# jorgeMFS/HYMET

Measured on AMD Instinct MI355X. Metric: contigs/s + Mbp/s classified, CAMI-medium, 1/2/4/8 MI355X; % HBM roofline, higher is better.
Workload: dtype u64

## Files before the change

hymet_amd/_lib.py:

```python
from __future__ import annotations

import ctypes
import os

HERE = os.path.dirname(os.path.abspath(__file__))
LIB_PATH = os.path.join(HERE, "libhymet_gpu.so")

_c = ctypes
_i64, _u64, _i32, _u32, _vp = _c.c_int64, _c.c_uint64, _c.c_int, _c.c_uint32, _c.c_void_p

_SIGS = {
    "hymet_version": (_i32, []),
    "hymet_init": (_i32, [_i32, _c.POINTER(_vp)]),
    "hymet_destroy": (_i32, [_vp]),
    "hymet_last_error": (_c.c_char_p, []),
    "hymet_set_stream": (_i32, [_vp, _vp]),
    "hymet_sync": (_i32, [_vp]),
    "hymet_prof_enable": (_i32, [_vp, _i32]),
    "hymet_prof_reset": (_i32, [_vp]),
    "hymet_prof_query": (_i32, [_vp, _c.c_char_p, _c.POINTER(_c.c_double), _c.POINTER(_i64), _c.POINTER(_c.c_double)]),
    "hymet_prof_names": (_i32, [_vp, _c.c_char_p, _i64]),
    "hymet_scratch_trim": (_i32, [_vp, _c.POINTER(_i64)]),
    "hymet_scratch_cached": (_i32, [_vp, _c.POINTER(_i64)]),
    "hymet_scratch_stats": (_i32, [_vp, _vp]),
# ... 42 lines not shown
    "hymet_paf_acc_create": (_i32, [_vp, _c.POINTER(_vp)]),
    "hymet_paf_acc_reset": (_i32, [_vp]),
    "hymet_paf_acc_destroy": (_i32, [_vp]),
    "hymet_paf_acc_info": (_i32, [_vp, _c.POINTER(_i64), _c.POINTER(_vp), _c.POINTER(_vp), _c.POINTER(_vp),
                                  _c.POINTER(_vp), _c.POINTER(_vp)]),
    "hymet_paf_acc_append": (_i32, [_vp, _vp, _vp, _i64, _i64]),
    "hymet_paf_acc_copy": (_i32, [_vp, _vp, _vp, _vp, _vp]),
    "hymet_paf_acc_field": (_i32, [_vp, _vp, _i32, _vp]),
    "hymet_mm_map_acc": (_i32, [_vp, _vp, _vp, _vp, _vp, _vp, _vp, _vp, _i32, _i32, _i32, _i32, _vp]),
    "hymet_emit_paf": (_i32, [_vp, _vp, _vp, _vp, _vp, _vp, _vp, _vp, _vp, _i64, _c.POINTER(_i64), _vp]),
    "hymet_acc_ref_counts": (_i32, [_vp, _vp, _vp]),
    "hymet_acc_classify": (_i32, [_vp, _vp, _i32, _i32] + [_vp] * 15 + [_c.POINTER(_i32)]),
    "hymet_emit_tsv": (_i32, [_vp, _i32, _i32] + [_vp] * 14 + [_i64, _c.POINTER(_i64)]),
    "hymet_mm_chain_dp": (_i32, [_vp, _vp, _vp, _i64, _i32, _i32, _i32, _i32, _i32, _c.c_float, _c.c_float, _vp, _vp]),
    "hymet_mm_mark_compact": (_i32, [_vp, _vp, _vp, _vp, _i64, _vp, _vp, _i32, _vp, _vp, _vp, _c.POINTER(_i64)]),
    "hymet_mm_anchor_sort": (_i32, [_vp, _vp, _vp, _i64, _vp, _i32, _i32, _i32, _u64, _i64, _vp, _vp, _vp, _vp, _vp]),
    "hymet_lca_ref_counts": (_i32, [_vp, _vp, _i64, _vp]),
    "hymet_lca": (_i32, [_vp, _i32, _i32] + [_vp] * 17),
}

_lib = None
_oom_hook = None


def _release_torch_cache(_user):
    try:
        import torch
        torch.cuda.empty_cache()
    except Exception:
        pass
# ... 134 lines not shown
```

hymet_amd/csrc/common.hpp:

```cpp
#pragma once
#include <hip/hip_runtime.h>
#include <stdint.h>
#include <algorithm>
#include <cstdlib>
#include <map>
#include <string>
#include <utility>
#include <vector>
#include "../../include/hymet_gpu.h"

struct hymet_ctx {
    int device = 0;
    hipStream_t stream = nullptr;
    bool own_stream = false;
    int n_cu = 256;
    bool prof = false;
    std::map<std::string, std::vector<std::pair<hipEvent_t, hipEvent_t>>> ev;
    std::map<std::string, double> bytes;
    std::map<std::string, std::pair<int, double>> dev_bytes;
    int64_t *prof_dev = nullptr;
    void *stage[2] = {nullptr, nullptr};
    hipEvent_t stage_ev[2] = {nullptr, nullptr};
    int64_t *mbox_h = nullptr;
    int64_t *mbox_d = nullptr;
    int32_t *dctr = nullptr;
};

namespace hymet {
struct ProfScope {
    hymet_ctx *c;
    const char *name;
    hipEvent_t a = nullptr, b = nullptr;
    ProfScope(hymet_ctx *ctx, const char *n, double alg_bytes = 0.0) : c(ctx), name(n) {
        if (c && c->prof && hipEventCreate(&a) == hipSuccess && hipEventCreate(&b) == hipSuccess) {
            (void)hipEventRecord(a, c->stream);
            c->bytes[name] += alg_bytes;
        }
    }
    ProfScope(hymet_ctx *ctx, const char *n, int slot, double per_unit) : ProfScope(ctx, n, 0.0) {
        if (c && c->prof) c->dev_bytes[name] = {slot, per_unit};
// ... 26 lines not shown
}
inline int64_t env_int(const char *name, int64_t dflt, int64_t lo, int64_t hi) {
    const char *e = env_str(name);
    return e ? std::max(lo, std::min(hi, (int64_t)atoll(e))) : dflt;
}
}

namespace hymet {
void set_error(const std::string &msg);
int fail(int code, const std::string &msg);
int hip_fail(hipError_t e, const char *what);
inline int64_t cdiv(int64_t a, int64_t b) { return (a + b - 1) / b; }
hipError_t scratch_alloc(size_t bytes, hipStream_t stream, void **p, size_t *cls);
void set_oom_hook(void (*hook)(void *), void *user);
void scratch_free(void *p, hipStream_t stream, size_t cls);
}

#define HY_CHECK_LAUNCH(what)                                   \
    do {                                                        \
        hipError_t e_ = hipGetLastError();                      \
        if (e_ != hipSuccess) return hymet::hip_fail(e_, what); \
    } while (0)

#define HY_HIP(call)                                            \
    do {                                                        \
        hipError_t e_ = (call);                                 \
        if (e_ != hipSuccess) return hymet::hip_fail(e_, #call); \
    } while (0)

#define HY_ARG(cond, msg)                                                   \
// ... 4 lines not shown
```

hymet_amd/csrc/ctx.cpp:

```cpp
#include "common.hpp"

#include <algorithm>
#include <thread>
#include <vector>

#include <cstring>
#include <map>
#include <mutex>
#include <tuple>
#include <cstdlib>
#include <vector>

namespace hymet {
static thread_local std::string g_err;
void set_error(const std::string &msg) { g_err = msg; }
int fail(int code, const std::string &msg) {
    g_err = msg;
    return code;
}
int hip_fail(hipError_t e, const char *what) {
    g_err = std::string(what) + ": " + hipGetErrorString(e);
    return HYMET_E_HIP;
}

// ... 98 lines not shown
    g_cache[{dev, stream, cls}].push_back(p);
    g_cached += cls;
}

int scratch_trim(int dev, int64_t *freed) {
    std::lock_guard<std::mutex> lk(g_cache_mu);
    const size_t before = g_cached;
    drop_cached(dev);
    if (freed) *freed = (int64_t)(before - g_cached);
    return HYMET_OK;
}

int64_t scratch_cached() {
    std::lock_guard<std::mutex> lk(g_cache_mu);
    return (int64_t)g_cached;
}

void scratch_stats(int64_t *out) {
    std::lock_guard<std::mutex> lk(g_cache_mu);
    for (int k = 0; k < 3; k++) out[k] = g_stats[k];
}
}

extern "C" {

int hymet_version(void) { return 1; }

const char *hymet_last_error(void) { return hymet::g_err.c_str(); }

int hymet_init(int device, hymet_ctx **out) {
// ... 27 lines not shown
        return hymet::fail(HYMET_E_HIP, "hymet_init: counter allocation failed");
    }
    *out = c;
    return HYMET_OK;
}

int hymet_destroy(hymet_ctx *ctx) {
    if (!ctx) return HYMET_OK;
    (void)hipSetDevice(ctx->device);
    for (int k = 0; k < 2; k++) {
        if (ctx->stage[k]) (void)hipHostFree(ctx->stage[k]);
        if (ctx->stage_ev[k]) (void)hipEventDestroy(ctx->stage_ev[k]);
    }
    if (ctx->mbox_h) (void)hipHostFree(ctx->mbox_h);
    if (ctx->dctr) (void)hipFree(ctx->dctr);
    if (ctx->prof_dev) (void)hipFree(ctx->prof_dev);
    if (ctx->own_stream && ctx->stream) (void)hipStreamDestroy(ctx->stream);
    delete ctx;
    return HYMET_OK;
}

int hymet_set_stream(hymet_ctx *ctx, void *s) {
    HY_ARG(ctx != nullptr, "hymet_set_stream: null ctx");
    HY_HIP(hipSetDevice(ctx->device));
    if (ctx->own_stream && ctx->stream) (void)hipStreamDestroy(ctx->stream);
    ctx->stream = (hipStream_t)s;
    ctx->own_stream = false;
    return HYMET_OK;
}

int hymet_prof_enable(hymet_ctx *ctx, int on) {
    HY_ARG(ctx != nullptr, "hymet_prof_enable: null ctx");
    ctx->prof = on != 0;
    return HYMET_OK;
}

int hymet_prof_reset(hymet_ctx *ctx) {
    HY_ARG(ctx != nullptr, "hymet_prof_reset: null ctx");
    HY_HIP(hipStreamSynchronize(ctx->stream));
// ... 36 lines not shown
}

int hymet_prof_names(hymet_ctx *ctx, char *buf, int64_t cap) {
    HY_ARG(ctx && buf && cap > 0, "hymet_prof_names: null argument");
    std::string all;
    for (auto &kv : ctx->ev) all += kv.first + "\n";
    if ((int64_t)all.size() + 1 > cap) return hymet::fail(HYMET_E_CAPACITY, "hymet_prof_names: buffer too small");
    memcpy(buf, all.c_str(), all.size() + 1);
    return HYMET_OK;
}

int hymet_scratch_trim(hymet_ctx *ctx, int64_t *freed_bytes) {
    HY_ARG(ctx != nullptr, "hymet_scratch_trim: null ctx");
    HY_HIP(hipSetDevice(ctx->device));
    HY_HIP(hipDeviceSynchronize());
    return hymet::scratch_trim(ctx->device, freed_bytes);
}

int hymet_scratch_reserve(hymet_ctx *ctx, int64_t bytes) {
    HY_ARG(ctx && bytes > 0, "hymet_scratch_reserve: bad argument");
    HY_HIP(hipSetDevice(ctx->device));
    void *p = nullptr;
    size_t cls = 0;
    HY_HIP(hymet::scratch_alloc((size_t)bytes, ctx->stream, &p, &cls));
    hymet::scratch_free(p, ctx->stream, cls);
    return HYMET_OK;
}

int hymet_set_oom_hook(void (*hook)(void *user), void *user) {
    hymet::set_oom_hook(hook, user);
// ... 91 lines not shown
```

hymet_amd/csrc/mm_chain.hip:

```cpp
#include "mm_common.hpp"

#include <cstdlib>
#include <string>

namespace hymet {
namespace mm {
namespace {

#ifndef HYMET_CHAIN_RING
#define HYMET_CHAIN_RING 128
#endif
#ifndef HYMET_CHAIN_SUMRING
#define HYMET_CHAIN_SUMRING 16
#endif
#ifndef HYMET_CHAIN_BDQ
#define HYMET_CHAIN_BDQ 32
#endif
#ifndef HYMET_CHAIN_IDQ
#define HYMET_CHAIN_IDQ 64
#endif
#ifndef HYMET_CHAIN_SPEC_GAP0
#define HYMET_CHAIN_SPEC_GAP0 2
#endif
#ifndef HYMET_CHAIN_WPE
// ... 1285 lines not shown
            ++i;
        }
        if (t_used) {
            __builtin_amdgcn_wave_barrier();
            for (int32_t j = lane; j < n; j += 64) P.t_global[g0 + j] = 0;
        }
        CPROF_FLUSH;
        GTIME_STOP;
    }
}

struct BacktrackParams {
    const int64_t *g_start;
    const int32_t *f;
    const int32_t *p;
    int32_t *t;
    const int32_t *z_cnt;
    const int32_t *z_idx;
    int32_t n_groups;
    int min_cnt, min_sc, max_drop;
    int64_t long_min;
    unsigned long long *prof;
    int32_t *chain_ids;
    uint64_t *chain_u;
    int64_t *chain_first;
    int32_t *n_chains;
};

constexpr int kBtWin = 8;

constexpr int64_t kBtLong = 64;
// ... 503 lines not shown
            hipLaunchKernelGGL(chain_work_anchors_kernel, dim3(wb), dim3(256), 0, st, P.g_start, P.order, P.n_work,
                               (const int32_t *)split.as<int32_t>(), pc);
            HY_CHECK_LAUNCH("chain_work_anchors_kernel");
        }
        P.work_end = split.as<int32_t>();
        if (long_pass) hipLaunchKernelGGL(chain_groups_kernel<1>, dim3((unsigned)blocks), dim3(64), kChainLds, st, P);
        else hipLaunchKernelGGL(chain_groups_kernel<0>, dim3((unsigned)blocks), dim3(64), kChainLds, st, P);
        HY_CHECK_LAUNCH("chain_groups_kernel");
    }
    ProfScope _pl(ctx, long_pass ? "mm_chain_long_small" : "mm_chain_small", slot + 1, 24.0);
    hipLaunchKernelGGL(chain_small_kernel, dim3((unsigned)cdiv(P.n_work, 64)), dim3(64), 0, st, P, (const int32_t *)split.as<int32_t>());
    HY_CHECK_LAUNCH("chain_small_kernel");
    return HYMET_OK;
}

int launch_backtrack(hymet_ctx *ctx, const int64_t *g_start, const int32_t *f, const int32_t *p, int32_t *t,
                     const int32_t *z_cnt, const int32_t *z_idx, int32_t n_groups, const int32_t *order, int32_t n_work,
                     int min_cnt, int min_sc, int max_drop, int32_t *chain_ids, uint64_t *chain_u, int64_t *chain_first,
                     int32_t *n_chains, int64_t n_anchors) {
    if (n_groups <= 0) return HYMET_OK;
    const int64_t long_min = env_int("HYMET_BT_LONG", kBtLong, 0, INT64_MAX);
    const bool prof = env_flag("HYMET_BT_PROF");
    DevBuf pbuf;
    if (prof) {
        HY_HIP(pbuf.alloc(64, ctx->stream));
        HY_HIP(hipMemsetAsync(pbuf.p, 0, 64, ctx->stream));
    }
    BacktrackParams P{g_start,  f,         p,       t,           z_cnt,    z_idx, n_groups, min_cnt, min_sc, max_drop,
                      long_min, (unsigned long long *)pbuf.p, chain_ids, chain_u, chain_first, n_chains};
    DevBuf cnt;
    HY_HIP(cnt.alloc(4 * (size_t)kBtCtrPad * (kBtStripes + 1), ctx->stream));
    ProfScope _ps(ctx, "mm_backtrack", 24.0 * (double)n_anchors);
    if (n_work > 0) {
        hipLaunchKernelGGL(bt_long_count_kernel, dim3(1), dim3(1), 0, ctx->stream, g_start, order, n_work, long_min,
                           cnt.as<int32_t>());
        HY_CHECK_LAUNCH("bt_long_count_kernel");
    }
    hipLaunchKernelGGL(backtrack_groups_kernel, dim3((unsigned)cdiv(n_groups, 64)), dim3(64), 0, ctx->stream, P);
    HY_CHECK_LAUNCH("backtrack_groups_kernel");
    if (n_work > 0) {
        ProfScope _pl(ctx, "mm_backtrack.long");
        const int per_cu = (int)env_int("HYMET_BT_WAVES", 24, 1, 1024);
        const int64_t nb = std::min<int64_t>(n_work, (int64_t)ctx->n_cu * per_cu);
        hipLaunchKernelGGL(backtrack_long_kernel, dim3((unsigned)nb), dim3(64), 0, ctx->stream, P, order,
                           cnt.as<int32_t>(), cnt.as<int32_t>() + kBtCtrPad);
        HY_CHECK_LAUNCH("backtrack_long_kernel");
    }
// ... 13 lines not shown
```

hymet_amd/csrc/mm_chainset.hip:

```cpp
#include "mm_stages.hpp"

#include <algorithm>
#include <cstdio>

namespace hymet {
namespace mm {

int launch_chain(hymet_ctx *ctx, const int32_t *ax, const uint32_t *ay, int span, const int64_t *g_start, const uint8_t *g_qfirst,
                 const int32_t *order, int32_t n_work, int32_t *f, int32_t *p, int32_t *t_global, int max_dist,
                 int max_dist_inner, int bw, int max_chn_skip, int cap_rmq_size, float pen_gap, float pen_skip,
                 int64_t n_anchors, int64_t n_groups);
int launch_backtrack(hymet_ctx *ctx, const int64_t *g_start, const int32_t *f, const int32_t *p, int32_t *t,
                     const int32_t *z_cnt, const int32_t *z_idx, int32_t n_groups, const int32_t *order, int32_t n_work,
                     int min_cnt, int min_sc, int max_drop, int32_t *chain_ids, uint64_t *chain_u, int64_t *chain_first,
                     int32_t *n_chains, int64_t n_anchors);

namespace {

constexpr int kGTile = 16384;

__device__ __forceinline__ uint64_t group_tile_bits(const uint32_t *hb, int64_t n, const int64_t *qoff, int n_q, int64_t t0,
                                                    uint64_t *qs) {
    __shared__ int s_q0;
    const int tid = threadIdx.x;
    const int64_t t1 = min(t0 + kGTile, n);
    const int64_t a0 = t0 + 64 * (int64_t)tid;
    const uint64_t hw = a0 < n ? reinterpret_cast<const uint64_t *>(hb)[a0 >> 6] : 0;
// ... 73 lines not shown
    if ((threadIdx.x & 63) == 0 && i < n) hb[i >> 6] = b;
}

__global__ void max_group_kernel(const int64_t *g_start, const int32_t *order, int32_t G, int64_t *out) {
    if (blockIdx.x != 0 || threadIdx.x != 0) return;
    int64_t best = 0;
    for (int32_t w = 0; w < G; w++) {
        const int g = order[w];
        const int64_t sz = g_start[g + 1] - g_start[g];
        best = max(best, sz);
        if (sz < 0xffff) break;
    }
    *out = best;
}

__global__ void nonwork_fp_kernel(const int64_t *g_start, int32_t G, int min_cnt, int32_t *f, int32_t *p, int32_t *t) {
    const int g = blockIdx.x * blockDim.x + threadIdx.x;
    if (g >= G) return;
    const int64_t a0 = g_start[g], a1 = g_start[g + 1];
    if (a1 - a0 >= min_cnt) return;
    for (int64_t a = a0; a < a1; a++) f[a] = 0, p[a] = -1, t[a] = 0;
}

__global__ void group_size_kernel(const int64_t *g_start, int32_t G, int min_cnt, uint32_t *key, uint32_t *gidx,
                                  uint32_t *is_work, uint8_t *qfirst, int32_t *zlists) {
    const int g = blockIdx.x * blockDim.x + threadIdx.x;
    if (g < 8) zlists[g] = 0;
    if (g >= G) return;
    if (qfirst) qfirst[g] = 0;
    const int64_t sz = g_start[g + 1] - g_start[g];
    key[g] = 0xffffu - (uint32_t)min(sz, (int64_t)0xffff);
    gidx[g] = (uint32_t)g;
    is_work[g] = sz >= min_cnt ? 1u : 0u;
}

constexpr int kZs = 2048;
// ... 408 lines not shown
        int64_t l2 = c, h2 = n_chain - 1;
        while (l2 < h2) {
            const int64_t mid = (l2 + h2 + 1) >> 1;
            if (bpos[mid] <= b) l2 = mid;
            else h2 = mid - 1;
        }
        c = l2;
    }
    const int32_t m = (int32_t)cu[c];
    const int64_t a = chain_ids[cfirst[c] + m - 1 - (b - bpos[c])];
    bx[b] = ax[a];
    by[b] = ay[a];
    bchain[b] = (int32_t)c;
}

__device__ __forceinline__ uint32_t keep_bits16(const int32_t *t, int64_t n, const uint32_t *qflag, const int64_t *qoff,
                                                int n_q, int64_t e0) {
    if (e0 >= n) return 0u;
    int lo = 0, hi = n_q - 1;
    while (lo < hi) {
        const int mid = (lo + hi + 1) >> 1;
        if (qoff[mid] <= e0) lo = mid;
        else hi = mid - 1;
    }
    int q = lo;
    int64_t qend = qoff[q + 1];
    int32_t v[16];
    if (e0 + 16 <= n) {
        const int4 *p4 = reinterpret_cast<const int4 *>(t + e0);
#pragma unroll
        for (int u = 0; u < 4; u++) {
            const int4 w = p4[u];
            v[4 * u] = w.x, v[4 * u + 1] = w.y, v[4 * u + 2] = w.z, v[4 * u + 3] = w.w;
        }
    } else {
#pragma unroll
        for (int u = 0; u < 16; u++) v[u] = e0 + u < n ? t[e0 + u] : 0;
    }
    uint32_t bits = 0, fl = qflag[q];
#pragma unroll
    for (int u = 0; u < 16; u++) {
        while (e0 + u >= qend && q + 1 < n_q) {
            q++;
            qend = qoff[q + 1];
            fl = qflag[q];
        }
        bits |= (uint32_t)(v[u] == 2 && fl != 0) << u;
    }
    return bits;
}

__global__ __launch_bounds__(256) void mark_count_kernel(const int32_t *t, int64_t n, const uint32_t *qflag,
                                                         const int64_t *qoff, int n_q, uint32_t *cnt, int64_t *last_kept) {
    __shared__ uint32_t ws[4];
    __shared__ int64_t wl[4];
    const int64_t e0 = (int64_t)blockIdx.x * 4096 + threadIdx.x * 16;
    const uint32_t kb = keep_bits16(t, n, qflag, qoff, n_q, e0);
    uint32_t c = __popc(kb);
    long long l = kb ? e0 + 31 - __clz((int)kb) : -1;
    for (int o = 32; o > 0; o >>= 1) {
        c += __shfl_xor((int)c, o, 64);
        l = max(l, __shfl_xor(l, o, 64));
    }
    if ((threadIdx.x & 63) == 0) ws[threadIdx.x >> 6] = c, wl[threadIdx.x >> 6] = l;
    __syncthreads();
    if (threadIdx.x == 0) {
        cnt[blockIdx.x] = ws[0] + ws[1] + ws[2] + ws[3];
        last_kept[blockIdx.x] = max(max(wl[0], wl[1]), max(wl[2], wl[3]));
    }
}

__global__ __launch_bounds__(256) void mark_compact_kernel(const int32_t *t, int64_t n, const uint32_t *qflag,
                                                           const int64_t *qoff, int n_q, const int64_t *tile_off,
                                                           const int64_t *last_kept, const uint64_t *ax, const uint32_t *ay,
                                                           uint64_t *ox, uint32_t *oy, uint32_t *ohb, uint32_t *ox32) {
    __shared__ uint32_t rc[64];
    __shared__ uint32_t nk[64];
    __shared__ uint32_t lx[64];
    __shared__ uint16_t kb[256];
    const int64_t t0 = (int64_t)blockIdx.x * 4096;
    const int lane = threadIdx.x & 63, w = threadIdx.x >> 6;
    kb[threadIdx.x] = (uint16_t)keep_bits16(t, n, qflag, qoff, n_q, t0 + threadIdx.x * 16);
    __syncthreads();
    bool m[16];
#pragma unroll
    for (int j = 0; j < 16; j++) {
        const int r = j * 256 + threadIdx.x;
// ... 143 lines not shown
            sidx.as<uint32_t>(), swork.as<uint32_t>(), (uint8_t *)nullptr, W.zlists.as<int32_t>());
    int rc = scan_flags(ctx, swork.as<uint32_t>(), G, wpos, &W.n_work);
    if (rc) return rc;
    uint32_t *kp = skey.as<uint32_t>(), *ka = skey2.as<uint32_t>(), *vp = sidx.as<uint32_t>(), *va = sidx2.as<uint32_t>();
    rc = sort_pairs(ctx, kp, ka, vp, va, G, 0, 16, "radix_sort_groups");
    if (rc) return rc;
    LAUNCH1(max_group_kernel, 1, Gr.g_start.as<int64_t>(), (const int32_t *)vp, (int32_t)G, mb_dev(ctx, kMbGmax));
    HY_HIP(hipStreamSynchronize(ctx->stream));
    W.largest = mb_read(ctx, kMbGmax);
    HY_ARG(W.largest < (1ll << 24) - 1, "chaining: an anchor group exceeds 2^24 anchors");
    W.order.swap(vp == sidx.as<uint32_t>() ? sidx : sidx2);
    return HYMET_OK;
}

static int chain_dp(hymet_ctx *ctx, const DpArgs &a, const AnchorSet &A, const Groups &Gr, const WorkList &W, DevBuf &f,
                    DevBuf &p, DevBuf &t) {
    HY_HIP(f.alloc(4 * (size_t)A.n, ctx->stream));
    HY_HIP(p.alloc(4 * (size_t)A.n, ctx->stream));
    LAUNCH1(nonwork_fp_kernel, Gr.G, Gr.g_start.as<int64_t>(), (int32_t)Gr.G, a.min_cnt, f.as<int32_t>(), p.as<int32_t>(),
            t.as<int32_t>());
    return launch_chain(ctx, A.ax32.as<int32_t>(), A.ay.as<uint32_t>(), A.span, Gr.g_start.as<int64_t>(), Gr.qfirst.as<uint8_t>(),
                        W.order.as<int32_t>(), (int32_t)W.n_work, f.as<int32_t>(), p.as<int32_t>(), t.as<int32_t>(), a.max_dist,
                        a.max_dist_inner, a.bw, a.max_chn_skip, a.cap_rmq_size, a.pen_gap, a.pen_skip, A.n, Gr.G);
}

static int z_order(hymet_ctx *ctx, int min_sc, const DevBuf &f, int64_t n, const Groups &Gr, const WorkList &W, ZOrder &Z) {
    const int64_t G = Gr.G;
    DevBuf zkey, z_runs, run_start, merge_list, mergeu_list, mid_list, big_list, big_off;
    HY_HIP(zkey.alloc(8 * (size_t)n, ctx->stream));
    HY_HIP(Z.idx.alloc(4 * (size_t)n, ctx->stream));
    HY_HIP(Z.cnt.alloc(4 * (size_t)G, ctx->stream));
    HY_HIP(z_runs.alloc(4 * (size_t)G, ctx->stream));
    HY_HIP(run_start.alloc(4 * (size_t)G * kZRuns, ctx->stream));
    HY_HIP(merge_list.alloc(4 * (size_t)G, ctx->stream));
    const int zm_lds = (int)env_int("HYMET_ZM_LDS", kZmLds, 0, kZmLds);
    const int zm_unit = (int)env_int("HYMET_ZM_UNIT", kZmUnit, 1, INT32_MAX);
    const int max_runs = (int)env_int("HYMET_Z_RUNS", kZRuns, 1, kZRuns);
// ... 39 lines not shown
    uint64_t *kp = sk.as<uint64_t>(), *ka = sk2.as<uint64_t>();
    uint32_t *vp = sv.as<uint32_t>(), *va = sv2.as<uint32_t>();
    rc = sort_pairs(ctx, kp, ka, vp, va, nz_big, 0, 32 + bits_for(n_big), "radix_sort_z_big");
    if (rc) return rc;
    hipLaunchKernelGGL(zbig_scatter_kernel, dim3((unsigned)n_big), dim3(256), 0, ctx->stream, P, (const uint32_t *)vp);
    HY_CHECK_LAUNCH("zbig_scatter_kernel");
    return HYMET_OK;
}

static int backtrack(hymet_ctx *ctx, const hymet_mm_opt *opt, int bw, int64_t n, const Groups &Gr, const WorkList &W,
                     const DevBuf &f, const DevBuf &p, DevBuf &t, const ZOrder &Z, Backtrack &B) {
    HY_HIP(B.ids.alloc(4 * (size_t)n, ctx->stream));
    HY_HIP(B.u.alloc(8 * (size_t)n, ctx->stream));
    HY_HIP(B.first.alloc(8 * (size_t)n, ctx->stream));
    HY_HIP(B.n_chains.alloc(4 * (size_t)Gr.G, ctx->stream));
    return launch_backtrack(ctx, Gr.g_start.as<int64_t>(), f.as<int32_t>(), p.as<int32_t>(), t.as<int32_t>(), Z.cnt.as<int32_t>(),
                            Z.idx.as<int32_t>(), (int32_t)Gr.G, W.order.as<int32_t>(), (int32_t)W.n_work, opt->min_cnt,
                            opt->min_chain_score, bw, B.ids.as<int32_t>(), B.u.as<uint64_t>(), B.first.as<int64_t>(),
                            B.n_chains.as<int32_t>(), n);
}

static int chain_list(hymet_ctx *ctx, const AnchorSet &A, int n_q, const Groups &Gr, const Backtrack &B, ChainSet &C,
                      DevBuf &cfirst) {
    const int64_t G = Gr.G;
    DevBuf cpos;
    int64_t NC = 0;
    int rc = scan_flags(ctx, (const uint32_t *)B.n_chains.p, G, cpos, &NC);
    if (rc) return rc;
    C.n_chain = NC;
    DevBuf ckey, cu, cf;
    HY_HIP(ckey.alloc(8 * (size_t)(NC + 1), ctx->stream));
// ... 74 lines not shown
    HY_ARG(n >= 0 && n < INT32_MAX, "chain_set: an anchor set of 2^31 anchors or more (32-bit chain links)");
    C.ax = A.ax.as<uint64_t>(), C.ay = A.ay.as<uint32_t>(), C.span = A.span;
    if (n == 0) {
        HY_HIP(C.d_qc.alloc(8 * (size_t)(n_q + 1), ctx->stream));
        HY_HIP(C.d_qb.alloc(8 * (size_t)(n_q + 1), ctx->stream));
        HY_HIP(hipMemsetAsync(C.d_qc.p, 0, 8 * (size_t)(n_q + 1), ctx->stream));
        HY_HIP(hipMemsetAsync(C.d_qb.p, 0, 8 * (size_t)(n_q + 1), ctx->stream));
        return HYMET_OK;
    }
    int rc = derive_heads(ctx, A);
    if (rc) return rc;
    Groups Gr;
    rc = build_groups(ctx, A, n_q, Gr);
    if (rc) return rc;
    DevBuf t;
    HY_HIP(t.alloc(4 * (size_t)n, ctx->stream));
    HY_HIP(hipMemsetAsync(t.p, 0, 4 * (size_t)n, ctx->stream));
    WorkList W;
    rc = build_work_list(ctx, Gr, opt->min_cnt, W);
    if (rc) return rc;
    if (env_flag("HYMET_CHAIN_STATS"))
        fprintf(stderr, "[chain] bw %d anchors %lld groups %lld work %lld largest %lld\n", bw, (long long)n, (long long)Gr.G,
                (long long)W.n_work, (long long)W.largest);
    DevBuf f, p;
    rc = chain_dp(ctx, DpArgs{opt->max_gap, opt->rmq_inner_dist, bw, opt->max_chain_skip, opt->rmq_size_cap, pen_gap, pen_skip,
                              opt->min_cnt}, A, Gr, W, f, p, t);
    if (rc) return rc;
    ZOrder Z;
    rc = z_order(ctx, opt->min_chain_score, f, n, Gr, W, Z);
    if (rc) return rc;
    Backtrack B;
    rc = backtrack(ctx, opt, bw, n, Gr, W, f, p, t, Z, B);
    if (rc) return rc;
    DevBuf cfirst;
    rc = chain_list(ctx, A, n_q, Gr, B, C, cfirst);
    if (rc) return rc;
    rc = chain_layout(ctx, A, n_q, B.ids, cfirst, C, lj, copy, t);
    if (rc) return rc;
    C.ids.swap(B.ids);
    C.cfirst.swap(cfirst);
    return HYMET_OK;
}

static int compact_marked(hymet_ctx *ctx, const AnchorSet &S1, const int32_t *mark, const uint32_t *flag, int n_q,
                          int64_t expect, AnchorSet &S2) {
    hipStream_t st = ctx->stream;
    const int64_t n1 = S1.n, nt = cdiv(n1, 4096);
    DevBuf tcnt, toff, tlast;
    HY_HIP(tcnt.alloc(4 * (size_t)(nt + 1), st));
    HY_HIP(toff.alloc(8 * (size_t)(nt + 1), st));
    HY_HIP(tlast.alloc(8 * (size_t)(nt + 1), st));
    hipLaunchKernelGGL(mark_count_kernel, dim3((unsigned)nt), dim3(256), 0, st, mark, n1, flag,
                       S1.d_off.as<int64_t>(), n_q, tcnt.as<uint32_t>(), tlast.as<int64_t>());
    HY_CHECK_LAUNCH("mark_count_kernel");
    int64_t A2 = 0;
    int rc = exclusive_scan_u32_i64(ctx, tcnt.as<uint32_t>(), toff.as<int64_t>(), nt, &A2);
    if (rc) return rc;
    if (expect >= 0 && A2 != expect) return hymet::fail(HYMET_E_INTERNAL, "hymet_mm_map: long-join anchor count mismatch");
    HY_HIP(S2.ax.alloc(8 * (size_t)(A2 + 1), st));
// ... 3 lines not shown
    HY_HIP(hipMemsetAsync(S2.hb.p, 0, head_bits_bytes(A2), st));
    hipLaunchKernelGGL(mark_compact_kernel, dim3((unsigned)nt), dim3(256), 0, st, mark, n1, flag,
                       S1.d_off.as<int64_t>(), n_q, toff.as<int64_t>(), tlast.as<int64_t>(), S1.ax.as<uint64_t>(),
                       S1.ay.as<uint32_t>(), S2.ax.as<uint64_t>(), S2.ay.as<uint32_t>(), S2.hb.as<uint32_t>(),
                       S2.ax32.as<uint32_t>());
    HY_CHECK_LAUNCH("mark_compact_kernel");
    S2.n = A2;
    S2.span = S1.span;
    S2.has_hb = S2.has_x32 = true;
    return HYMET_OK;
}

int marked_anchor_set(hymet_ctx *ctx, const AnchorSet &S1, const LeanJoin &lj, const uint32_t *flag, int n_q, int64_t A2,
                      AnchorSet &S2) {
    if (A2 != lj.n2) return hymet::fail(HYMET_E_INTERNAL, "hymet_mm_map: long-join anchor count mismatch");
    return compact_marked(ctx, S1, lj.mark.as<int32_t>(), flag, n_q, A2, S2);
}

static int narrow_y(const uint64_t *h_y, int64_t n, std::vector<uint32_t> &y32, int *span, const char *what) {
    y32.resize((size_t)n);
    for (int64_t i = 0; i < n; i++) {
        if ((h_y[i] >> 32) != (h_y[0] >> 32)) return hymet::fail(HYMET_E_ARG, what);
        y32[(size_t)i] = (uint32_t)h_y[i];
    }
    *span = n > 0 ? (int)(h_y[0] >> 32 & 0xff) : 0;
    return HYMET_OK;
}

}
}

// ... 16 lines not shown
    if (rc) return rc;
    HY_HIP(A.ax.alloc(8 * (size_t)n, st));
    HY_HIP(A.ay.alloc(4 * (size_t)n, st));
    HY_HIP(A.d_off.alloc(sizeof h_off, st));
    HY_HIP(hipMemcpyAsync(A.ax.p, h_x, 8 * (size_t)n, hipMemcpyHostToDevice, st));
    HY_HIP(hipMemcpyAsync(A.ay.p, y32.data(), 4 * (size_t)n, hipMemcpyHostToDevice, st));
    HY_HIP(hipMemcpyAsync(A.d_off.p, h_off, sizeof h_off, hipMemcpyHostToDevice, st));
    rc = derive_heads(ctx, A);
    if (rc) return rc;
    Groups Gr;
    rc = build_groups(ctx, A, 1, Gr);
    if (rc) return rc;
    WorkList W;
    rc = build_work_list(ctx, Gr, 1, W);
    if (rc) return rc;
    DevBuf f, p, t;
    HY_HIP(t.alloc(4 * (size_t)n, st));
    HY_HIP(hipMemsetAsync(t.p, 0, 4 * (size_t)n, st));
    rc = chain_dp(ctx, DpArgs{max_dist, max_dist_inner, bw, max_chn_skip, cap_rmq_size, pen_gap, pen_skip, 1}, A, Gr, W, f, p, t);
    if (rc) return rc;
    HY_HIP(hipMemcpyAsync(h_f, f.p, 4 * (size_t)n, hipMemcpyDeviceToHost, st));
    std::vector<int32_t> p32((size_t)n);
    HY_HIP(hipMemcpyAsync(p32.data(), p.p, 4 * (size_t)n, hipMemcpyDeviceToHost, st));
    HY_HIP(hipStreamSynchronize(st));
    for (int64_t i = 0; i < n; i++) h_p[i] = p32[(size_t)i];
    return HYMET_OK;
}

extern "C" int hymet_mm_mark_compact(hymet_ctx *ctx, const uint64_t *h_x, const uint64_t *h_y, const int32_t *h_mark, int64_t n,
                                     const int64_t *h_qoff, const uint32_t *h_qflag, int32_t n_q, uint64_t *h_ox,
                                     uint64_t *h_oy, uint32_t *h_ohb, int64_t *n_kept) {
    HY_ARG(ctx && h_x && h_y && h_mark && h_qoff && h_qflag && h_ox && h_oy && h_ohb && n_kept,
           "hymet_mm_mark_compact: null argument");
    HY_ARG(n > 0 && n < INT32_MAX && n_q > 0, "hymet_mm_mark_compact: n or n_q out of range");
    HY_ARG(h_qoff[0] == 0 && h_qoff[n_q] == n, "hymet_mm_mark_compact: query offsets do not span the anchors");
    for (int32_t q = 0; q < n_q; q++) HY_ARG(h_qoff[q] <= h_qoff[q + 1], "hymet_mm_mark_compact: query offsets not rising");
    HY_HIP(hipSetDevice(ctx->device));
    hipStream_t st = ctx->stream;
    AnchorSet S1, S2;
    S1.n = n;
    std::vector<uint32_t> y32;
    int rc = narrow_y(h_y, n, y32, &S1.span, "hymet_mm_mark_compact: the anchors' y values carry different spans");
    if (rc) return rc;
    DevBuf mark, flag;
    HY_HIP(S1.ax.alloc(8 * (size_t)n, st));
    HY_HIP(S1.ay.alloc(4 * (size_t)n, st));
    HY_HIP(S1.d_off.alloc(8 * (size_t)(n_q + 1), st));
    HY_HIP(mark.alloc(4 * (size_t)n + 16, st));
    HY_HIP(flag.alloc(4 * (size_t)n_q, st));
    HY_HIP(hipMemcpyAsync(S1.ax.p, h_x, 8 * (size_t)n, hipMemcpyHostToDevice, st));
    HY_HIP(hipMemcpyAsync(S1.ay.p, y32.data(), 4 * (size_t)n, hipMemcpyHostToDevice, st));
    HY_HIP(hipMemcpyAsync(S1.d_off.p, h_qoff, 8 * (size_t)(n_q + 1), hipMemcpyHostToDevice, st));
    HY_HIP(hipMemcpyAsync(mark.p, h_mark, 4 * (size_t)n, hipMemcpyHostToDevice, st));
    HY_HIP(hipMemcpyAsync(flag.p, h_qflag, 4 * (size_t)n_q, hipMemcpyHostToDevice, st));
    rc = compact_marked(ctx, S1, mark.as<int32_t>(), flag.as<uint32_t>(), n_q, -1, S2);
    if (rc) {
        HY_HIP(hipStreamSynchronize(st));
        return rc;
    }
    const int64_t m = S2.n;
    std::vector<uint32_t> oy32((size_t)m);
    if (m > 0) {
        HY_HIP(hipMemcpyAsync(h_ox, S2.ax.p, 8 * (size_t)m, hipMemcpyDeviceToHost, st));
        HY_HIP(hipMemcpyAsync(oy32.data(), S2.ay.p, 4 * (size_t)m, hipMemcpyDeviceToHost, st));
        HY_HIP(hipMemcpyAsync(h_ohb, S2.hb.p, 4 * (size_t)((m + 31) / 32), hipMemcpyDeviceToHost, st));
    }
    HY_HIP(hipStreamSynchronize(st));
    for (int64_t i = 0; i < m; i++) h_oy[i] = (h_y[0] >> 32) << 32 | oy32[(size_t)i];
    *n_kept = m;
    return HYMET_OK;
// ... 2 lines not shown
```

include/hymet_gpu.h:

```cpp
#ifndef HYMET_GPU_H
#define HYMET_GPU_H

#include <stdint.h>

#ifdef __cplusplus
extern "C" {
#endif

#define HYMET_OK 0
#define HYMET_E_HIP (-1)
#define HYMET_E_ARG (-2)
#define HYMET_E_CAPACITY (-3)
#define HYMET_E_INTERNAL (-4)

typedef struct hymet_ctx hymet_ctx;

int hymet_init(int device, hymet_ctx **out);
int hymet_destroy(hymet_ctx *ctx);
const char *hymet_last_error(void);
int hymet_set_stream(hymet_ctx *ctx, void *hip_stream);
int hymet_sync(hymet_ctx *ctx);
int hymet_version(void);
int hymet_prof_enable(hymet_ctx *ctx, int on);
int hymet_prof_reset(hymet_ctx *ctx);
// ... 128 lines not shown
int hymet_paf_acc_append(hymet_ctx *ctx, hymet_paf_acc *dst, const hymet_paf_acc *src, int64_t begin, int64_t end);
int hymet_paf_acc_copy(hymet_ctx *ctx, const hymet_paf_acc *acc, int32_t *h_q, int32_t *h_part, int32_t *h_t);
int hymet_paf_acc_field(hymet_ctx *ctx, const hymet_paf_acc *acc, int field, int32_t *h_out);
int hymet_mm_map_acc(hymet_ctx *ctx, const hymet_mm_index *idx, const hymet_mm_opt *opt, const uint32_t *d_2b,
                     const uint32_t *d_mask, const int64_t *h_starts, const int64_t *h_lens, const uint32_t *d_name_hash,
                     int32_t n_q, int32_t q_base, int32_t part_id, int32_t t_base, hymet_paf_acc *acc);
int hymet_emit_paf(hymet_ctx *ctx, const hymet_paf_acc *acc, const uint8_t *d_qname, const int64_t *d_qname_off,
                   const int64_t *d_qlen, const uint8_t *d_tname, const int64_t *d_tname_off, const int64_t *d_tlen,
                   char *d_out, int64_t cap, int64_t *n_bytes, int64_t *d_line_off);
int hymet_mm_chain_dp(hymet_ctx *ctx, const uint64_t *h_x, const uint64_t *h_y, int64_t n, int max_dist,
                      int max_dist_inner, int bw, int max_chn_skip, int cap_rmq_size, float pen_gap,
                      float pen_skip, int32_t *h_f, int64_t *h_p);
int hymet_mm_mark_compact(hymet_ctx *ctx, const uint64_t *h_x, const uint64_t *h_y, const int32_t *h_mark, int64_t n,
                          const int64_t *h_qoff, const uint32_t *h_qflag, int32_t n_q, uint64_t *h_ox, uint64_t *h_oy,
                          uint32_t *h_ohb, int64_t *n_kept);
int hymet_mm_anchor_sort(hymet_ctx *ctx, const uint64_t *h_key, const uint32_t *h_val, int64_t n,
                         const int64_t *h_qoff, int32_t n_q, int32_t rb, int32_t pb, uint64_t yhi, int64_t max_qlen,
                         uint64_t *h_ax, uint64_t *h_ay, uint32_t *h_ax32, uint32_t *h_hb, int64_t *h_stats);

int hymet_lca_ref_counts(hymet_ctx *ctx, const int32_t *d_line_t, int64_t n_lines, int32_t *d_counts);
int hymet_acc_ref_counts(hymet_ctx *ctx, const hymet_paf_acc *acc, int32_t *d_counts);
int hymet_acc_classify(hymet_ctx *ctx, const hymet_paf_acc *acc, int mode, int32_t n_q, const int64_t *d_qlen,
                       const int32_t *d_ref_counts, const int32_t *d_t_tax, const int32_t *d_tax_names,
                       const uint8_t *d_tax_in_hier, const uint8_t *d_qname_pool, const int64_t *d_qname_off,
                       const uint8_t *d_tname_pool, const int64_t *d_tname_off, int32_t *d_row_q, int32_t *d_row_part,
                       int32_t *d_row_depth, int32_t *d_row_names, double *d_row_conf, int32_t *d_row_tax,
                       int32_t *n_rows);
int hymet_emit_tsv(hymet_ctx *ctx, int mode, int32_t n_rows, const int32_t *d_row_q, const int32_t *d_row_depth,
                   const int32_t *d_row_names, const double *d_row_conf, const int32_t *d_row_tax, const uint8_t *d_qname,
                   const int64_t *d_qname_off, const uint8_t *d_label, const int64_t *d_label_off, const uint8_t *d_taxlin,
// ... 14 lines not shown
```

Before: 134,000.

## Split chain DP scratch into persistent stamp buffer and byte-wide mark array

The per-anchor t array was a 32-bit buffer allocated and zeroed on every call, and it served both as DP scratch and as the backtrack/compaction mark. The DP now gets a persistent per-context int32 stamp buffer that is zeroed only when it grows, while the mark becomes a uint8 array read 16 at a time with one uint4 load in the compaction kernels. This is meant to cut per-call allocation, memset and mark read/write traffic. It relies on the chain kernel restoring the stamp buffer to zero after use, and it adds lifetime handling on stream change, trim and destroy plus a debug query for nonzero stamp entries.

Result: faster. 136,300, median of 6 (+1.7%).

```diff
diff --git a/hymet_amd/_lib.py b/hymet_amd/_lib.py
--- a/hymet_amd/_lib.py
+++ b/hymet_amd/_lib.py
@@ -80,6 +80,7 @@
     "hymet_emit_tsv": (_i32, [_vp, _i32, _i32] + [_vp] * 14 + [_i64, _c.POINTER(_i64)]),
     "hymet_mm_chain_dp": (_i32, [_vp, _vp, _vp, _i64, _i32, _i32, _i32, _i32, _i32, _c.c_float, _c.c_float, _vp, _vp]),
     "hymet_mm_mark_compact": (_i32, [_vp, _vp, _vp, _vp, _i64, _vp, _vp, _i32, _vp, _vp, _vp, _c.POINTER(_i64)]),
+    "hymet_mm_stamp_scratch": (_i32, [_vp, _c.POINTER(_i64), _c.POINTER(_i64)]),
     "hymet_mm_anchor_sort": (_i32, [_vp, _vp, _vp, _i64, _vp, _i32, _i32, _i32, _u64, _i64, _vp, _vp, _vp, _vp, _vp]),
     "hymet_lca_ref_counts": (_i32, [_vp, _vp, _i64, _vp]),
     "hymet_lca": (_i32, [_vp, _i32, _i32] + [_vp] * 17),
diff --git a/hymet_amd/csrc/common.hpp b/hymet_amd/csrc/common.hpp
--- a/hymet_amd/csrc/common.hpp
+++ b/hymet_amd/csrc/common.hpp
@@ -24,6 +24,9 @@
     int64_t *mbox_h = nullptr;
     int64_t *mbox_d = nullptr;
     int32_t *dctr = nullptr;
+    int32_t *stamp = nullptr;
+    int64_t stamp_cap = 0;
+    size_t stamp_cls = 0;
 };
 
 namespace hymet {
@@ -80,6 +83,8 @@
 hipError_t scratch_alloc(size_t bytes, hipStream_t stream, void **p, size_t *cls);
 void set_oom_hook(void (*hook)(void *), void *user);
 void scratch_free(void *p, hipStream_t stream, size_t cls);
+hipError_t stamp_scratch(hymet_ctx *ctx, int64_t n, int32_t **out);
+void stamp_release(hymet_ctx *ctx);
 }
 
 #define HY_CHECK_LAUNCH(what)                                   \
diff --git a/hymet_amd/csrc/ctx.cpp b/hymet_amd/csrc/ctx.cpp
--- a/hymet_amd/csrc/ctx.cpp
+++ b/hymet_amd/csrc/ctx.cpp
@@ -136,6 +136,33 @@
 int64_t scratch_cached() {
     std::lock_guard<std::mutex> lk(g_cache_mu);
     return (int64_t)g_cached;
+}
+
+hipError_t stamp_scratch(hymet_ctx *ctx, int64_t n, int32_t **out) {
+    if (n > ctx->stamp_cap) {
+        stamp_release(ctx);
+        void *p = nullptr;
+        size_t cls = 0;
+        hipError_t e = scratch_alloc(4 * (size_t)n, ctx->stream, &p, &cls);
+        if (e != hipSuccess) return e;
+        e = hipMemsetAsync(p, 0, cls, ctx->stream);
+        if (e != hipSuccess) {
+            scratch_free(p, ctx->stream, cls);
+            return e;
+        }
+        ctx->stamp = (int32_t *)p;
+        ctx->stamp_cap = (int64_t)(cls / 4);
+        ctx->stamp_cls = cls;
+    }
+    *out = ctx->stamp;
+    return hipSuccess;
+}
+
+void stamp_release(hymet_ctx *ctx) {
+    if (ctx->stamp) scratch_free(ctx->stamp, ctx->stream, ctx->stamp_cls);
+    ctx->stamp = nullptr;
+    ctx->stamp_cap = 0;
+    ctx->stamp_cls = 0;
 }
 
 void scratch_stats(int64_t *out) {
@@ -193,6 +220,7 @@
     }
     if (ctx->mbox_h) (void)hipHostFree(ctx->mbox_h);
     if (ctx->dctr) (void)hipFree(ctx->dctr);
+    if (ctx->stamp) (void)hipFree(ctx->stamp);
     if (ctx->prof_dev) (void)hipFree(ctx->prof_dev);
     if (ctx->own_stream && ctx->stream) (void)hipStreamDestroy(ctx->stream);
     delete ctx;
@@ -202,6 +230,10 @@
 int hymet_set_stream(hymet_ctx *ctx, void *s) {
     HY_ARG(ctx != nullptr, "hymet_set_stream: null ctx");
     HY_HIP(hipSetDevice(ctx->device));
+    if (ctx->stamp) {
+        HY_HIP(hipStreamSynchronize(ctx->stream));
+        hymet::stamp_release(ctx);
+    }
     if (ctx->own_stream && ctx->stream) (void)hipStreamDestroy(ctx->stream);
     ctx->stream = (hipStream_t)s;
     ctx->own_stream = false;
@@ -268,6 +300,7 @@
     HY_ARG(ctx != nullptr, "hymet_scratch_trim: null ctx");
     HY_HIP(hipSetDevice(ctx->device));
     HY_HIP(hipDeviceSynchronize());
+    hymet::stamp_release(ctx);
     return hymet::scratch_trim(ctx->device, freed_bytes);
 }
 
diff --git a/hymet_amd/csrc/mm_chain.hip b/hymet_amd/csrc/mm_chain.hip
--- a/hymet_amd/csrc/mm_chain.hip
+++ b/hymet_amd/csrc/mm_chain.hip
@@ -1323,7 +1323,7 @@
     const int64_t *g_start;
     const int32_t *f;
     const int32_t *p;
-    int32_t *t;
+    uint8_t *t;
     const int32_t *z_cnt;
     const int32_t *z_idx;
     int32_t n_groups;
@@ -1857,7 +1857,7 @@
     return HYMET_OK;
 }
 
-int launch_backtrack(hymet_ctx *ctx, const int64_t *g_start, const int32_t *f, const int32_t *p, int32_t *t,
+int launch_backtrack(hymet_ctx *ctx, const int64_t *g_start, const int32_t *f, const int32_t *p, uint8_t *t,
                      const int32_t *z_cnt, const int32_t *z_idx, int32_t n_groups, const int32_t *order, int32_t n_work,
                      int min_cnt, int min_sc, int max_drop, int32_t *chain_ids, uint64_t *chain_u, int64_t *chain_first,
                      int32_t *n_chains, int64_t n_anchors) {
@@ -1873,7 +1873,7 @@
                       long_min, (unsigned long long *)pbuf.p, chain_ids, chain_u, chain_first, n_chains};
     DevBuf cnt;
     HY_HIP(cnt.alloc(4 * (size_t)kBtCtrPad * (kBtStripes + 1), ctx->stream));
-    ProfScope _ps(ctx, "mm_backtrack", 24.0 * (double)n_anchors);
+    ProfScope _ps(ctx, "mm_backtrack", 18.0 * (double)n_anchors);
     if (n_work > 0) {
         hipLaunchKernelGGL(bt_long_count_kernel, dim3(1), dim3(1), 0, ctx->stream, g_start, order, n_work, long_min,
                            cnt.as<int32_t>());
diff --git a/hymet_amd/csrc/mm_chainset.hip b/hymet_amd/csrc/mm_chainset.hip
--- a/hymet_amd/csrc/mm_chainset.hip
+++ b/hymet_amd/csrc/mm_chainset.hip
@@ -10,7 +10,7 @@
                  const int32_t *order, int32_t n_work, int32_t *f, int32_t *p, int32_t *t_global, int max_dist,
                  int max_dist_inner, int bw, int max_chn_skip, int cap_rmq_size, float pen_gap, float pen_skip,
                  int64_t n_anchors, int64_t n_groups);
-int launch_backtrack(hymet_ctx *ctx, const int64_t *g_start, const int32_t *f, const int32_t *p, int32_t *t,
+int launch_backtrack(hymet_ctx *ctx, const int64_t *g_start, const int32_t *f, const int32_t *p, uint8_t *t,
                      const int32_t *z_cnt, const int32_t *z_idx, int32_t n_groups, const int32_t *order, int32_t n_work,
                      int min_cnt, int min_sc, int max_drop, int32_t *chain_ids, uint64_t *chain_u, int64_t *chain_first,
                      int32_t *n_chains, int64_t n_anchors);
@@ -114,12 +114,15 @@
     *out = best;
 }
 
-__global__ void nonwork_fp_kernel(const int64_t *g_start, int32_t G, int min_cnt, int32_t *f, int32_t *p, int32_t *t) {
+__global__ void nonwork_fp_kernel(const int64_t *g_start, int32_t G, int min_cnt, int32_t *f, int32_t *p, uint8_t *t) {
     const int g = blockIdx.x * blockDim.x + threadIdx.x;
     if (g >= G) return;
     const int64_t a0 = g_start[g], a1 = g_start[g + 1];
     if (a1 - a0 >= min_cnt) return;
-    for (int64_t a = a0; a < a1; a++) f[a] = 0, p[a] = -1, t[a] = 0;
+    for (int64_t a = a0; a < a1; a++) {
+        f[a] = 0, p[a] = -1;
+        if (t) t[a] = 0;
+    }
 }
 
 __global__ void group_size_kernel(const int64_t *g_start, int32_t G, int min_cnt, uint32_t *key, uint32_t *gidx,
@@ -558,7 +561,7 @@
     bchain[b] = (int32_t)c;
 }
 
-__device__ __forceinline__ uint32_t keep_bits16(const int32_t *t, int64_t n, const uint32_t *qflag, const int64_t *qoff,
+__device__ __forceinline__ uint32_t keep_bits16(const uint8_t *t, int64_t n, const uint32_t *qflag, const int64_t *qoff,
                                                 int n_q, int64_t e0) {
     if (e0 >= n) return 0u;
     int lo = 0, hi = n_q - 1;
@@ -569,17 +572,13 @@
     }
     int q = lo;
     int64_t qend = qoff[q + 1];
-    int32_t v[16];
+    uint32_t v[4] = {0, 0, 0, 0};
     if (e0 + 16 <= n) {
-        const int4 *p4 = reinterpret_cast<const int4 *>(t + e0);
-#pragma unroll
-        for (int u = 0; u < 4; u++) {
-            const int4 w = p4[u];
-            v[4 * u] = w.x, v[4 * u + 1] = w.y, v[4 * u + 2] = w.z, v[4 * u + 3] = w.w;
-        }
+        const uint4 w = *reinterpret_cast<const uint4 *>(t + e0);
+        v[0] = w.x, v[1] = w.y, v[2] = w.z, v[3] = w.w;
     } else {
 #pragma unroll
-        for (int u = 0; u < 16; u++) v[u] = e0 + u < n ? t[e0 + u] : 0;
+        for (int u = 0; u < 16; u++) v[u >> 2] |= (e0 + u < n ? (uint32_t)t[e0 + u] : 0u) << (8 * (u & 3));
     }
     uint32_t bits = 0, fl = qflag[q];
 #pragma unroll
@@ -589,12 +588,12 @@
             qend = qoff[q + 1];
             fl = qflag[q];
         }
-        bits |= (uint32_t)(v[u] == 2 && fl != 0) << u;
+        bits |= (uint32_t)((v[u >> 2] >> (8 * (u & 3)) & 0xffu) == 2u && fl != 0) << u;
     }
     return bits;
 }
 
-__global__ __launch_bounds__(256) void mark_count_kernel(const int32_t *t, int64_t n, const uint32_t *qflag,
+__global__ __launch_bounds__(256) void mark_count_kernel(const uint8_t *t, int64_t n, const uint32_t *qflag,
                                                          const int64_t *qoff, int n_q, uint32_t *cnt, int64_t *last_kept) {
     __shared__ uint32_t ws[4];
     __shared__ int64_t wl[4];
@@ -614,7 +613,7 @@
     }
 }
 
-__global__ __launch_bounds__(256) void mark_compact_kernel(const int32_t *t, int64_t n, const uint32_t *qflag,
+__global__ __launch_bounds__(256) void mark_compact_kernel(const uint8_t *t, int64_t n, const uint32_t *qflag,
                                                            const int64_t *qoff, int n_q, const int64_t *tile_off,
                                                            const int64_t *last_kept, const uint64_t *ax, const uint32_t *ay,
                                                            uint64_t *ox, uint32_t *oy, uint32_t *ohb, uint32_t *ox32) {
@@ -788,13 +787,15 @@
 }
 
 static int chain_dp(hymet_ctx *ctx, const DpArgs &a, const AnchorSet &A, const Groups &Gr, const WorkList &W, DevBuf &f,
-                    DevBuf &p, DevBuf &t) {
+                    DevBuf &p, uint8_t *mark) {
     HY_HIP(f.alloc(4 * (size_t)A.n, ctx->stream));
     HY_HIP(p.alloc(4 * (size_t)A.n, ctx->stream));
+    int32_t *stamp = nullptr;
+    HY_HIP(stamp_scratch(ctx, A.n, &stamp));
     LAUNCH1(nonwork_fp_kernel, Gr.G, Gr.g_start.as<int64_t>(), (int32_t)Gr.G, a.min_cnt, f.as<int32_t>(), p.as<int32_t>(),
-            t.as<int32_t>());
+            mark);
     return launch_chain(ctx, A.ax32.as<int32_t>(), A.ay.as<uint32_t>(), A.span, Gr.g_start.as<int64_t>(), Gr.qfirst.as<uint8_t>(),
-                        W.order.as<int32_t>(), (int32_t)W.n_work, f.as<int32_t>(), p.as<int32_t>(), t.as<int32_t>(), a.max_dist,
+                        W.order.as<int32_t>(), (int32_t)W.n_work, f.as<int32_t>(), p.as<int32_t>(), stamp, a.max_dist,
                         a.max_dist_inner, a.bw, a.max_chn_skip, a.cap_rmq_size, a.pen_gap, a.pen_skip, A.n, Gr.G);
 }
 
@@ -864,7 +865,7 @@
     HY_HIP(B.u.alloc(8 * (size_t)n, ctx->stream));
     HY_HIP(B.first.alloc(8 * (size_t)n, ctx->stream));
     HY_HIP(B.n_chains.alloc(4 * (size_t)Gr.G, ctx->stream));
-    return launch_backtrack(ctx, Gr.g_start.as<int64_t>(), f.as<int32_t>(), p.as<int32_t>(), t.as<int32_t>(), Z.cnt.as<int32_t>(),
+    return launch_backtrack(ctx, Gr.g_start.as<int64_t>(), f.as<int32_t>(), p.as<int32_t>(), t.as<uint8_t>(), Z.cnt.as<int32_t>(),
                             Z.idx.as<int32_t>(), (int32_t)Gr.G, W.order.as<int32_t>(), (int32_t)W.n_work, opt->min_cnt,
                             opt->min_chain_score, bw, B.ids.as<int32_t>(), B.u.as<uint64_t>(), B.first.as<int64_t>(),
                             B.n_chains.as<int32_t>(), n);
@@ -969,8 +970,8 @@
     rc = build_groups(ctx, A, n_q, Gr);
     if (rc) return rc;
     DevBuf t;
-    HY_HIP(t.alloc(4 * (size_t)n, ctx->stream));
-    HY_HIP(hipMemsetAsync(t.p, 0, 4 * (size_t)n, ctx->stream));
+    HY_HIP(t.alloc((size_t)n + 16, ctx->stream));
+    HY_HIP(hipMemsetAsync(t.p, 0, (size_t)n + 16, ctx->stream));
     WorkList W;
     rc = build_work_list(ctx, Gr, opt->min_cnt, W);
     if (rc) return rc;
@@ -979,7 +980,7 @@
                 (long long)W.n_work, (long long)W.largest);
     DevBuf f, p;
     rc = chain_dp(ctx, DpArgs{opt->max_gap, opt->rmq_inner_dist, bw, opt->max_chain_skip, opt->rmq_size_cap, pen_gap, pen_skip,
-                              opt->min_cnt}, A, Gr, W, f, p, t);
+                              opt->min_cnt}, A, Gr, W, f, p, t.as<uint8_t>());
     if (rc) return rc;
     ZOrder Z;
     rc = z_order(ctx, opt->min_chain_score, f, n, Gr, W, Z);
@@ -997,7 +998,7 @@
     return HYMET_OK;
 }
 
-static int compact_marked(hymet_ctx *ctx, const AnchorSet &S1, const int32_t *mark, const uint32_t *flag, int n_q,
+static int compact_marked(hymet_ctx *ctx, const AnchorSet &S1, const uint8_t *mark, const uint32_t *flag, int n_q,
                           int64_t expect, AnchorSet &S2) {
     hipStream_t st = ctx->stream;
     const int64_t n1 = S1.n, nt = cdiv(n1, 4096);
@@ -1031,7 +1032,7 @@
 int marked_anchor_set(hymet_ctx *ctx, const AnchorSet &S1, const LeanJoin &lj, const uint32_t *flag, int n_q, int64_t A2,
                       AnchorSet &S2) {
     if (A2 != lj.n2) return hymet::fail(HYMET_E_INTERNAL, "hymet_mm_map: long-join anchor count mismatch");
-    return compact_marked(ctx, S1, lj.mark.as<int32_t>(), flag, n_q, A2, S2);
+    return compact_marked(ctx, S1, lj.mark.as<uint8_t>(), flag, n_q, A2, S2);
 }
 
 static int narrow_y(const uint64_t *h_y, int64_t n, std::vector<uint32_t> &y32, int *span, const char *what) {
@@ -1078,16 +1079,46 @@
     WorkList W;
     rc = build_work_list(ctx, Gr, 1, W);
     if (rc) return rc;
-    DevBuf f, p, t;
-    HY_HIP(t.alloc(4 * (size_t)n, st));
-    HY_HIP(hipMemsetAsync(t.p, 0, 4 * (size_t)n, st));
-    rc = chain_dp(ctx, DpArgs{max_dist, max_dist_inner, bw, max_chn_skip, cap_rmq_size, pen_gap, pen_skip, 1}, A, Gr, W, f, p, t);
+    DevBuf f, p;
+    rc = chain_dp(ctx, DpArgs{max_dist, max_dist_inner, bw, max_chn_skip, cap_rmq_size, pen_gap, pen_skip, 1}, A, Gr, W, f, p,
+                  nullptr);
     if (rc) return rc;
     HY_HIP(hipMemcpyAsync(h_f, f.p, 4 * (size_t)n, hipMemcpyDeviceToHost, st));
     std::vector<int32_t> p32((size_t)n);
     HY_HIP(hipMemcpyAsync(p32.data(), p.p, 4 * (size_t)n, hipMemcpyDeviceToHost, st));
     HY_HIP(hipStreamSynchronize(st));
     for (int64_t i = 0; i < n; i++) h_p[i] = p32[(size_t)i];
+    return HYMET_OK;
+}
+
+namespace {
+__global__ __launch_bounds__(256) void stamp_nonzero_kernel(const int32_t *t, int64_t n, unsigned long long *out) {
+    unsigned long long c = 0;
+    for (int64_t i = (int64_t)blockIdx.x * 256 + threadIdx.x; i < n; i += (int64_t)gridDim.x * 256) c += t[i] != 0;
+    for (int o = 32; o > 0; o >>= 1) c += __shfl_xor(c, o, 64);
+    if ((threadIdx.x & 63) == 0 && c) atomicAdd(out, c);
+}
+}
+
+extern "C" int hymet_mm_stamp_scratch(hymet_ctx *ctx, int64_t *capacity, int64_t *nonzero) {
+    HY_ARG(ctx && capacity && nonzero, "hymet_mm_stamp_scratch: null argument");
+    HY_HIP(hipSetDevice(ctx->device));
+    hipStream_t st = ctx->stream;
+    HY_HIP(hipStreamSynchronize(st));
+    *capacity = ctx->stamp_cap;
+    *nonzero = 0;
+    if (ctx->stamp_cap == 0) return HYMET_OK;
+    DevBuf cnt;
+    HY_HIP(cnt.alloc(8, st));
+    HY_HIP(hipMemsetAsync(cnt.p, 0, 8, st));
+    const int64_t nb = std::min<int64_t>(cdiv(ctx->stamp_cap, 256), (int64_t)ctx->n_cu * 8);
+    hipLaunchKernelGGL(stamp_nonzero_kernel, dim3((unsigned)nb), dim3(256), 0, st, (const int32_t *)ctx->stamp, ctx->stamp_cap,
+                       cnt.as<unsigned long long>());
+    HY_CHECK_LAUNCH("stamp_nonzero_kernel");
+    unsigned long long h = 0;
+    HY_HIP(hipMemcpyAsync(&h, cnt.p, 8, hipMemcpyDeviceToHost, st));
+    HY_HIP(hipStreamSynchronize(st));
+    *nonzero = (int64_t)h;
     return HYMET_OK;
 }
 
@@ -1110,14 +1141,16 @@
     HY_HIP(S1.ax.alloc(8 * (size_t)n, st));
     HY_HIP(S1.ay.alloc(4 * (size_t)n, st));
     HY_HIP(S1.d_off.alloc(8 * (size_t)(n_q + 1), st));
-    HY_HIP(mark.alloc(4 * (size_t)n + 16, st));
+    std::vector<uint8_t> m8((size_t)n);
+    for (int64_t i = 0; i < n; i++) m8[(size_t)i] = h_mark[i] == 2 ? 2 : (h_mark[i] != 0);
+    HY_HIP(mark.alloc((size_t)n + 16, st));
     HY_HIP(flag.alloc(4 * (size_t)n_q, st));
     HY_HIP(hipMemcpyAsync(S1.ax.p, h_x, 8 * (size_t)n, hipMemcpyHostToDevice, st));
     HY_HIP(hipMemcpyAsync(S1.ay.p, y32.data(), 4 * (size_t)n, hipMemcpyHostToDevice, st));
     HY_HIP(hipMemcpyAsync(S1.d_off.p, h_qoff, 8 * (size_t)(n_q + 1), hipMemcpyHostToDevice, st));
-    HY_HIP(hipMemcpyAsync(mark.p, h_mark, 4 * (size_t)n, hipMemcpyHostToDevice, st));
+    HY_HIP(hipMemcpyAsync(mark.p, m8.data(), (size_t)n, hipMemcpyHostToDevice, st));
     HY_HIP(hipMemcpyAsync(flag.p, h_qflag, 4 * (size_t)n_q, hipMemcpyHostToDevice, st));
-    rc = compact_marked(ctx, S1, mark.as<int32_t>(), flag.as<uint32_t>(), n_q, -1, S2);
+    rc = compact_marked(ctx, S1, mark.as<uint8_t>(), flag.as<uint32_t>(), n_q, -1, S2);
     if (rc) {
         HY_HIP(hipStreamSynchronize(st));
         return rc;
diff --git a/include/hymet_gpu.h b/include/hymet_gpu.h
--- a/include/hymet_gpu.h
+++ b/include/hymet_gpu.h
@@ -166,6 +166,7 @@
 int hymet_mm_mark_compact(hymet_ctx *ctx, const uint64_t *h_x, const uint64_t *h_y, const int32_t *h_mark, int64_t n,
                           const int64_t *h_qoff, const uint32_t *h_qflag, int32_t n_q, uint64_t *h_ox, uint64_t *h_oy,
                           uint32_t *h_ohb, int64_t *n_kept);
+int hymet_mm_stamp_scratch(hymet_ctx *ctx, int64_t *capacity, int64_t *nonzero);
 int hymet_mm_anchor_sort(hymet_ctx *ctx, const uint64_t *h_key, const uint32_t *h_val, int64_t n,
                          const int64_t *h_qoff, int32_t n_q, int32_t rb, int32_t pb, uint64_t yhi, int64_t max_qlen,
                          uint64_t *h_ax, uint64_t *h_ay, uint32_t *h_ax32, uint32_t *h_hb, int64_t *h_stats);
```
